# thegedge/StereoReconstruction

Hardware: AMD Instinct MI355X
Metric: Mdisparity-hypotheses/s (WxHxD) (higher is better)
Workload: dtype f64; 1 GPU; C3: synthetic rectified 1920x1080 pair, 256 depth levels, GeodesicWeight r=5; TwoView WTA both directions + cross-check; one pair per GPU; width=1920, height=1080, depth_levels=256, window_radius=5, weights=geodesic, pairs_per_gpu=1, pair_seed_rank0=1592590339, pair_seed_of_rank_r=seed + 0x10000*r, parallelism=single GPU

## Files before the change

stereoreconstruction_amd/csrc/srh_block.hpp:

```cpp
#pragma once

#include <math.h>

#if defined(__HIPCC__)
#include <hip/hip_runtime.h>
#endif
#ifndef SRH_NHD
#if defined(__HIPCC__)
#define SRH_NHD __host__ __device__ __forceinline__
#else
#define SRH_NHD inline
#endif
#endif
#if defined(__HIP_DEVICE_COMPILE__)
#define SRH_SCHED_BARRIER() __builtin_amdgcn_sched_barrier(0)
#define SRH_LDS_WAIT() __builtin_amdgcn_s_waitcnt(0xC07F)
#else
#define SRH_SCHED_BARRIER() do { } while (0)
#define SRH_LDS_WAIT() do { } while (0)
#endif

namespace srh {

template <int WS, int NCB, bool FMA, class Src>
SRH_NHD void block_two_sweeps(const Src src, int ra, int rb, double mL, double tw, double (&sum1)[NCB], double (&sum3)[NCB])
{
	constexpr int NR = NCB + WS - 1;
	static_assert(WS % 2 == 1 && NR % 2 == 0, "odd window, the other view's segment in pairs");
	double r[NR], wv[WS], acc[NCB];
	{
		const auto first = src.row(ra);
#pragma unroll
		for (int m = 0; m < NR/2; ++m) first.r2(m, r[2*m], r[2*m + 1]);
#pragma unroll
		for (int m = 0; m < (WS - 1)/2; ++m) first.w2(m, wv[2*m], wv[2*m + 1]);
		wv[WS - 1] = first.w(WS - 1);
	}
#pragma unroll
	for (int j = 0; j < NCB; ++j) acc[j] = 0.0;
	if (Src::LDS_WAIT) SRH_LDS_WAIT();
#pragma unroll 1
	for (int row = ra; row < rb; ++row) {
		const int seen = src.row_begin(1);
		const auto next = src.row(row + 1 < rb ? row + 1 : ra);
#pragma unroll
		for (int col = 0; col < WS; ++col) {
			if (FMA) {
#pragma unroll
				for (int j = 0; j < NCB; ++j) acc[j] = __builtin_fma(wv[col], r[col + j], acc[j]);
			} else {
				double pr[NCB];
#pragma unroll
				for (int j = 0; j < NCB; ++j) pr[j] = wv[col]*r[col + j];
				SRH_SCHED_BARRIER();
#pragma unroll
				for (int j = 0; j < NCB; ++j) acc[j] += pr[j];
			}
			SRH_SCHED_BARRIER();
			if (col & 1) {
				next.r2(col >> 1, r[col - 1], r[col]);
				next.w2(col >> 1, wv[col - 1], wv[col]);
				SRH_SCHED_BARRIER();
			}
		}
#pragma unroll
		for (int m = (WS - 1)/2; m < NR/2; ++m) next.r2(m, r[2*m], r[2*m + 1]);
		wv[WS - 1] = next.w(WS - 1);
		src.row_end(seen);
	}
	double mR[NCB], s1[NCB], s3[NCB], av[WS];
	{
		const auto first = src.row(ra);
#pragma unroll
		for (int col = 0; col < WS; ++col) av[col] = first.l(col);
	}
#pragma unroll
	for (int j = 0; j < NCB; ++j) { mR[j] = acc[j]/tw; s1[j] = 0.0; s3[j] = 0.0; }
	if (Src::LDS_WAIT) SRH_LDS_WAIT();
#pragma unroll 1
	for (int row = ra; row < rb; ++row) {
		const int seen = src.row_begin(3);
		const auto next = src.row(row + 1 < rb ? row + 1 : ra);
#pragma unroll
		for (int col = 0; col < WS; ++col) {
			const double wt = wv[col];
			if (FMA) {
				const double a = __builtin_fma(wt, av[col], -mL);
				double bb[NCB];
#pragma unroll
				for (int j = 0; j < NCB; ++j) bb[j] = __builtin_fma(wt, r[col + j], -mR[j]);
				SRH_SCHED_BARRIER();
#pragma unroll
				for (int j = 0; j < NCB; ++j) { s1[j] = __builtin_fma(a, bb[j], s1[j]); s3[j] = __builtin_fma(bb[j], bb[j], s3[j]); }
			} else {
				double bb[NCB], u1[NCB], u3[NCB];
				const double pa = wt*av[col];
#pragma unroll
				for (int j = 0; j < NCB; ++j) bb[j] = wt*r[col + j];
				SRH_SCHED_BARRIER();
				const double a = pa - mL;
#pragma unroll
				for (int j = 0; j < NCB; ++j) bb[j] = bb[j] - mR[j];
				SRH_SCHED_BARRIER();
#pragma unroll
				for (int j = 0; j < NCB; ++j) { u1[j] = a*bb[j]; u3[j] = bb[j]*bb[j]; }
				SRH_SCHED_BARRIER();
#pragma unroll
				for (int j = 0; j < NCB; ++j) { s1[j] += u1[j]; s3[j] += u3[j]; }
			}
			SRH_SCHED_BARRIER();
			av[col] = next.l(col);
			if (col & 1) {
				next.r2(col >> 1, r[col - 1], r[col]);
				next.w2(col >> 1, wv[col - 1], wv[col]);
			}
			SRH_SCHED_BARRIER();
		}
#pragma unroll
		for (int m = (WS - 1)/2; m < NR/2; ++m) next.r2(m, r[2*m], r[2*m + 1]);
		wv[WS - 1] = next.w(WS - 1);
		src.row_end(seen);
	}
#pragma unroll
	for (int j = 0; j < NCB; ++j) { sum1[j] = s1[j]; sum3[j] = s3[j]; }
}

template <int WS, int NCB, class Src>
SRH_NHD void block_onepass(const Src src, double mL, double (&Pout)[NCB], double (&Qout)[NCB], double (&Uout)[NCB])
{
	double P[NCB], Q[NCB], U[NCB];
	constexpr int NR = NCB + WS - 1;
	static_assert(WS % 2 == 1 && NR % 2 == 0, "odd window, the other view's segment in pairs");
	double r[NR], q[NR], wv[WS], lv[WS];
	{
		const auto first = src.row(0);
#pragma unroll
		for (int m = 0; m < NR/2; ++m) first.r2(m, r[2*m], r[2*m + 1]);
#pragma unroll
		for (int m = 0; m < (WS - 1)/2; ++m) first.w2(m, wv[2*m], wv[2*m + 1]);
		wv[WS - 1] = first.w(WS - 1);
#pragma unroll
		for (int col = 0; col < WS; ++col) lv[col] = first.l(col);
	}
#pragma unroll
	for (int j = 0; j < NCB; ++j) { P[j] = 0.0; Q[j] = 0.0; U[j] = 0.0; }
	if (Src::LDS_WAIT) SRH_LDS_WAIT();
#pragma unroll 1
	for (int row = 0; row < WS; ++row) {
		const int seen = src.row_begin(4);
		const auto next = src.row(row + 1 < WS ? row + 1 : 0);
#pragma unroll
		for (int k = 0; k < NCB - 1; ++k) q[k] = r[k]*r[k];
#pragma unroll
		for (int col = 0; col < WS; ++col) {
			q[col + NCB - 1] = r[col + NCB - 1]*r[col + NCB - 1];
			const double a = __builtin_fma(wv[col], lv[col], -mL);
			const double c = a*wv[col], d = wv[col]*wv[col];
			SRH_SCHED_BARRIER();
#pragma unroll
			for (int j = 0; j < NCB; ++j) P[j] = __builtin_fma(wv[col], r[col + j], P[j]);
#pragma unroll
			for (int j = 0; j < NCB; ++j) Q[j] = __builtin_fma(c, r[col + j], Q[j]);
#pragma unroll
			for (int j = 0; j < NCB; ++j) U[j] = __builtin_fma(d, q[col + j], U[j]);
			SRH_SCHED_BARRIER();
			lv[col] = next.l(col);
			if (col & 1) {
				next.r2(col >> 1, r[col - 1], r[col]);
				next.w2(col >> 1, wv[col - 1], wv[col]);
			}
			SRH_SCHED_BARRIER();
		}
#pragma unroll
		for (int m = (WS - 1)/2; m < NR/2; ++m) next.r2(m, r[2*m], r[2*m + 1]);
		wv[WS - 1] = next.w(WS - 1);
		src.row_end(seen);
	}
#pragma unroll
	for (int j = 0; j < NCB; ++j) { Pout[j] = P[j]; Qout[j] = Q[j]; Uout[j] = U[j]; }
}

SRH_NHD double two_sweep_finish(double s1, double s2, double s3) { return 255*(1.0 - fabs(s1) / sqrt(s2 * s3)); }

SRH_NHD double rsq_seed(double x)
{
#if defined(__HIP_DEVICE_COMPILE__)
	return __builtin_amdgcn_rsq(x);
#else
	return 1.0/sqrt(x);
#endif
}

SRH_NHD double onepass_finish(double P, double Q, double U, double SA, double itw, double s2, double TT,
                              double sig3, double zmax2, bool &okc)
{
	const double m = P*itw, p2 = P + P;
	const double s3 = __builtin_fma(-m, __builtin_fma(-TT, m, p2), U);
	const double s1 = __builtin_fma(-m, SA, Q);
	const double q3 = __builtin_fma(m, __builtin_fma(TT, m, p2), U);
	const double x = s2*s3;
	const double y0 = rsq_seed(x);
	const double e = __builtin_fma(-(x*y0), y0, 1.0);
	const double y1 = __builtin_fma(y0*e, __builtin_fma(0.375, e, 0.5), y0);
	const bool c1 = s3 >= sig3, c2 = s3*zmax2 >= q3, c3 = __builtin_fabs(e) <= 0x1p-20;
	okc = c1 & c2 & c3;
	return __builtin_fma(-255.0, __builtin_fabs(s1)*y1, 255.0);
}

template <bool CERT, class B = double>
SRH_NHD double block_stored(double v, bool certified, B m_hi, B clamp)
{
	if (CERT) return !certified ? __builtin_nan("") : (v > m_hi ? clamp : v);
	return (v < clamp) ? v : clamp;
}

}
```

stereoreconstruction_amd/csrc/srh_strip.hip:

```cpp
#include "srh_internal.hpp"
#include "srh_geom.hpp"
#include "srh_walk.hpp"
#include "srh_block.hpp"

#include <type_traits>

namespace srh {

#ifdef SRH_EXPERIMENT
__device__ int g_strip_exp_repeat = 1;
void strip_exp_set(int repeat) { (void)hipMemcpyToSymbol(HIP_SYMBOL(g_strip_exp_repeat), &repeat, sizeof(int)); }
#endif

#define ST_TP 32
#define ST_NCB 8
#define ST_CHUNK 320
#define ST_BROWS 1

typedef __attribute__((address_space(3))) void st_lds_void;
typedef __attribute__((address_space(1))) const void st_gbl_void;
typedef __attribute__((address_space(3))) volatile int st_lds_vint;

__global__ void padded_plane_kernel(const double *__restrict__ gray_tv, int W, int H, double *__restrict__ out)
{
	const int SP = padded_stride(W), HP = H + 2*SRH_PADY;
	const size_t n = (size_t)SP*HP;
	const double nan = __builtin_nan("");
	for (size_t k = (size_t)blockIdx.x*blockDim.x + threadIdx.x; k < n; k += (size_t)gridDim.x*blockDim.x) {
		const int x = (int)(k % (size_t)SP) - SRH_PADL, y = (int)(k / (size_t)SP) - SRH_PADY;
		out[k] = (x >= 0 && y >= 0 && x < W && y < H) ? gray_tv[(size_t)y*W + x] : nan;
	}
}

void launch_padded_plane(hipStream_t st, const double *gray_tv, int w, int h, double *out) {
	size_t n = padded_size(w, h);
	size_t b = (n + 255)/256; if (b > 4096) b = 4096;
	hipLaunchKernelGGL(padded_plane_kernel, dim3((unsigned)b), dim3(256), 0, st, gray_tv, w, h, out);
}

__global__ void padded_full_kernel(const double *__restrict__ gray_tv, int W, int H, int R, uint8_t *__restrict__ out)
{
	const int SP = padded_stride(W), HP = H + 2*SRH_PADY;
	const size_t n = (size_t)SP*HP;
	for (size_t k = (size_t)blockIdx.x*blockDim.x + threadIdx.x; k < n; k += (size_t)gridDim.x*blockDim.x) {
		const int x = (int)(k % (size_t)SP) - SRH_PADL, y = (int)(k / (size_t)SP) - SRH_PADY;
		bool ok = x - R >= 0 && y - R >= 0 && x + R < W && y + R < H;
		for (int row = -R; ok && row <= R; ++row)
			for (int col = -R; col <= R; ++col) {
				const double v = gray_tv[(size_t)(y + row)*W + (x + col)];
				ok = ok && (v == v);
			}
		out[k] = ok ? 1 : 0;
	}
}

void launch_padded_full(hipStream_t st, const double *gray_tv, int w, int h, int R, uint8_t *out) {
	size_t n = padded_size(w, h);
	size_t b = (n + 255)/256; if (b > 4096) b = 4096;
	hipLaunchKernelGGL(padded_full_kernel, dim3((unsigned)b), dim3(256), 0, st, gray_tv, w, h, R, out);
}

__global__ void pixel_range_kernel(const ViewDev *__restrict__ views, int ref, int oth, srh_params P, int y0, int nrows,
                                   const double *__restrict__ tnum, int cstride, PixRange *__restrict__ prange,
                                   int ncb, int lanes, int pad, uint32_t *__restrict__ filllist)
{
	const ViewDev &L = views[ref];
	const int W = L.w;
	const size_t q = (size_t)blockIdx.x*blockDim.x + threadIdx.x;
	const bool in = q < (size_t)nrows*W;
	int lo = 0, hi = -1;
	if (in) {
		const int x = (int)(q % W), y = y0 + (int)(q / W);
		if (L.mask[(size_t)y*W + x] == 1) {
			const Ray ray = cam_unproject(L.cam, (x + 0.5) / P.image_scale, (y + 0.5) / P.image_scale);
			pinhole_column_range(ray, L.cam, views[oth], P, tnum, cstride, lo, hi);
		}
		PixRange r; r.lo = lo; r.hi = hi;
		prange[q] = r;
	}
	if (!filllist) return;
	const bool left = in && hi >= lo && dense_cover_hi(lo, hi, ncb, lanes, pad != 0) < hi;
	const unsigned long long m = __ballot(left);
	if (m == 0) return;
	const int lane = (int)(threadIdx.x & 63), leader = __ffsll((long long)m) - 1;
	unsigned base = 0;
	if (lane == leader) base = atomicAdd(&filllist[0], (unsigned)__popcll(m));
	base = (unsigned)__shfl((int)base, leader);
	if (left) filllist[1 + base + (unsigned)__popcll(m & ((1ull << lane) - 1ull))] = (uint32_t)q;
}

void launch_pixel_range(hipStream_t st, const ViewDev *views, int ref, int oth, int width, const srh_params &P,
                        int y0, int nrows, const double *tnum, int cstride, PixRange *prange,
                        int lanes, bool padded, uint32_t *filllist)
{
	const size_t n = (size_t)nrows*width;
	hipLaunchKernelGGL(pixel_range_kernel, dim3((unsigned)((n + 255)/256)), dim3(256), 0, st,
	                   views, ref, oth, P, y0, nrows, tnum, cstride, prange, 8, lanes, padded ? 1 : 0, filllist);
}

int strip_chunk_columns() { return ST_CHUNK; }

struct StripArgs {
	int W, H, y0, nrows;
	const double *wimg;
	const double *pconst;
	const PixRange *prange;
	const double *ref_tvp, *oth_tvp;
	const uint8_t *oth_fullp;
	double *cost; int cstride;
	Counters *cnt;
	int n1, n2;
	int nitems;
	double weight_cutoff, bad_ret, max_color_diff;
	CertBound cb;
	int redo;
};

static void strip_items(StripArgs &a) {
	a.n1 = ((a.nrows*3/4)/16)*16;
	a.n2 = a.n1 + (((a.nrows - a.n1)*2/3)/8)*8;
	const int nseg = a.n1/16 + (a.n2 - a.n1)/8 + (a.nrows - a.n2 + 3)/4;
	a.nitems = nseg*((a.W + ST_TP - 1)/ST_TP);
}

template <int R, int NBUF>
struct StripSmem {
	static constexpr int WS = 2*R + 1;
	static constexpr int T = WS*WS;
	static constexpr int WP = (WS + 1) & ~1;
	static constexpr int WPIX = WS*WP;
	static constexpr int RW = ST_CHUNK + 2*R + ST_NCB + 2;
	static constexpr int LW = (ST_TP + 2*R + 1) & ~1;
	static constexpr int NS = WS + 1;
	static constexpr int FW = (RW + 4 + 15) & ~15;
	static constexpr int NBMAX = ST_CHUNK/ST_NCB + 1;
	static constexpr int GL_CAP = 3072;
	static constexpr int GL_SINGLES = GL_CAP - ST_TP*NBMAX;
	alignas(16) double w[NBUF][WS][ST_TP][WP];
	alignas(16) double rt[NS][RW];
	alignas(16) double rto[NBUF == 2 ? NS : 1][RW];
	alignas(16) double lt[NS][LW];
	alignas(16) double pc[2][ST_TP][SRH_PC];
	alignas(16) PixRange pr[2][ST_TP];
	alignas(16) unsigned char full[2][FW];
	unsigned short glist[GL_CAP];
	int glist_n, gsingle_n;
	int item;
	unsigned long long badcols[ST_CHUNK/64 + 2];
	int simd[8];
	int prog[NBUF == 2 ? 8 : 1][64];
	static_assert(ST_CHUNK <= 512 && ST_TP <= 64, "work-list entry = pixel*512 + column in 16 bits");
	static_assert(RW % 2 == 0 && LW % 2 == 0 && WP % 2 == 0, "16-byte rows");
	static_assert(RW - R + 4 <= SRH_PADR + 1, "padded planes cover every staged piece");
};

__device__ __forceinline__ void st_dma16(const void *src, void *dst, int nbytes, int lane) {
	for (int off = 0; off < nbytes; off += 1024) {
		if (off + lane*16 < nbytes)
			__builtin_amdgcn_global_load_lds((st_gbl_void *)((const char *)src + off + lane*16),
			                                 (st_lds_void *)((char *)dst + off), 16, 0, 0);
	}
}
__device__ __forceinline__ void st_dma4(const void *src, void *dst, int nbytes, int lane) {
	for (int off = 0; off < nbytes; off += 256) {
		if (off + lane*4 < nbytes)
			__builtin_amdgcn_global_load_lds((st_gbl_void *)((const char *)src + off + lane*4),
			                                 (st_lds_void *)((char *)dst + off), 4, 0, 0);
	}
}

template <int R, int NBUF>
__device__ __noinline__ double strip_cost_general(const StripSmem<R, NBUF> &S, int wb, int s0, int i, int rc,
                                                  double weight_cutoff, double bad_ret, double max_color_diff)
{
	typedef StripSmem<R, NBUF> Smem;
	constexpr int WS = Smem::WS, NS = Smem::NS;
	return ncc_select_cost<WS>([&](int row, double *gl, double *gr, double *wt) {
		const int sl = s0 + row >= NS ? s0 + row - NS : s0 + row;
#pragma unroll
		for (int col = 0; col < WS; ++col) { gl[col] = S.lt[sl][i + col]; gr[col] = S.rt[sl][rc + col]; wt[col] = S.w[wb][row][i][col]; }
	}, weight_cutoff, bad_ret, max_color_diff);
}

template <int R, int NBUF>
__device__ __noinline__ void strip_select_block(const StripSmem<R, NBUF> &S, int wb, int s0, int pi, int rc, unsigned store,
                                                double *__restrict__ dst, double weight_cutoff, double bad_ret, double max_color_diff,
                                                int ra, int rb)
{
	typedef StripSmem<R, NBUF> Smem;
	constexpr int WS = Smem::WS, NS = Smem::NS, NCB = ST_NCB, NR = NCB + 2*R;
	double mLs[NCB], mRs[NCB], tws[NCB];
#pragma unroll
	for (int j = 0; j < NCB; ++j) { mLs[j] = 0.0; mRs[j] = 0.0; tws[j] = 0.0; }
#pragma unroll 1
	for (int row = ra; row < rb; ++row) {
		const int sl = s0 + row >= NS ? s0 + row - NS : s0 + row;
		double rr[NR], rv[NR];
		const double2 *rp = reinterpret_cast<const double2 *>((NBUF == 2 && (rc & 1)) ? &S.rto[sl][rc - 1] : &S.rt[sl][rc]);
#pragma unroll
		for (int m = 0; m < NR/2; ++m) { const double2 v = rp[m]; rr[2*m] = v.x; rr[2*m + 1] = v.y; }
#pragma unroll
		for (int m = 0; m < NR; ++m) { const bool okr = rr[m] == rr[m]; rv[m] = okr ? 1.0 : 0.0; rr[m] = okr ? rr[m] : 0.0; }
#pragma unroll
		for (int col = 0; col < WS; ++col) {
			const double gl = S.lt[sl][pi + col], wt = S.w[wb][row][pi][col];
			const bool okl = gl == gl && wt > weight_cutoff;
			const double w0 = okl ? wt : 0.0, pl0 = okl ? wt*gl : 0.0;
#pragma unroll
			for (int j = 0; j < NCB; ++j) {
				mLs[j] += pl0*rv[col + j];
				mRs[j] += w0*rr[col + j];
				tws[j] += w0*rv[col + j];
			}
		}
	}
#pragma unroll
	for (int j = 0; j < NCB; ++j) { mLs[j] /= tws[j]; mRs[j] /= tws[j]; }
	double s1[NCB], s2v[NCB], s3[NCB];
#pragma unroll
	for (int j = 0; j < NCB; ++j) { s1[j] = 0.0; s2v[j] = 0.0; s3[j] = 0.0; }
#pragma unroll 1
	for (int row = ra; row < rb; ++row) {
		const int sl = s0 + row >= NS ? s0 + row - NS : s0 + row;
		double rr[NR], rv[NR];
		const double2 *rp = reinterpret_cast<const double2 *>((NBUF == 2 && (rc & 1)) ? &S.rto[sl][rc - 1] : &S.rt[sl][rc]);
#pragma unroll
		for (int m = 0; m < NR/2; ++m) { const double2 v = rp[m]; rr[2*m] = v.x; rr[2*m + 1] = v.y; }
#pragma unroll
		for (int m = 0; m < NR; ++m) { const bool okr = rr[m] == rr[m]; rv[m] = okr ? 1.0 : 0.0; rr[m] = okr ? rr[m] : 0.0; }
#pragma unroll
		for (int col = 0; col < WS; ++col) {
			const double gl = S.lt[sl][pi + col], wt = S.w[wb][row][pi][col];
			const bool okl = gl == gl && wt > weight_cutoff;
			const double pl = wt*(gl == gl ? gl : 0.0), kl = okl ? 1.0 : 0.0;
#pragma unroll
			for (int j = 0; j < NCB; ++j) {
				const double k = kl*rv[col + j];
				const double a = (pl - mLs[j])*k, bq = (wt*rr[col + j] - mRs[j])*k;
				s1[j] += a*bq;
				s2v[j] += a*a;
				s3[j] += bq*bq;
			}
		}
	}
#pragma unroll
	for (int j = 0; j < NCB; ++j) {
		if ((store >> j) & 1u) {
			double result = bad_ret;
			if (!(tws[j] < 1e-10)) {
				const double v = 255*(1.0 - fabs(s1[j]) / sqrt(s2v[j] * s3[j]));
				result = (v < max_color_diff) ? v : max_color_diff;
			}
			dst[(ptrdiff_t)j*ST_TP] = result;
		}
	}
}

template <int R, int NWV, int NBUF>
struct StripRows {
	typedef StripSmem<R, NBUF> Smem;
	static constexpr bool LDS_WAIT = true;
	Smem &S;
	const double *rbase;
	int s0, wb, i, rc, wv, lane, partner;
	int &prog;
	struct Row {
		const double2 *rp, *wp;
		const double *lp;
		__device__ __forceinline__ void r2(int m, double &a, double &b) const { const double2 v = rp[m]; a = v.x; b = v.y; }
		__device__ __forceinline__ void w2(int m, double &a, double &b) const { const double2 v = wp[m]; a = v.x; b = v.y; }
		__device__ __forceinline__ double w(int col) const { return reinterpret_cast<const double *>(wp)[col]; }
		__device__ __forceinline__ double l(int col) const { return lp[col]; }
	};
	__device__ __forceinline__ Row row(int row) const {
		const int sl = s0 + row >= Smem::NS ? s0 + row - Smem::NS : s0 + row;
		return Row{ reinterpret_cast<const double2 *>(rbase + sl*Smem::RW + rc), reinterpret_cast<const double2 *>(&S.w[wb][row][i][0]), &S.lt[sl][i] };
	}
	__device__ __forceinline__ int row_begin(int units) const {
		int seen = 0;
		if (NWV == 8) {
			prog += units;
			*(st_lds_vint *)&S.prog[wv][lane] = prog;
			seen = *(st_lds_vint *)&S.prog[partner][lane];
		}
		return seen;
	}
	__device__ __forceinline__ void row_end(int seen) const {
		if (NWV == 8) {
			const int ps = __builtin_amdgcn_readfirstlane(seen), pm = __builtin_amdgcn_readfirstlane(prog);
			asm volatile("s_nop 0\n\ts_cmp_gt_i32 %0, %1\n\ts_cbranch_scc1 1f\n\ts_setprio 1\n\ts_branch 2f\n1:\n\ts_setprio 0\n2:"
			             :: "s"(pm), "s"(ps) : "scc");
		}
	}
};

template <int R, int NWV, int NBUF, int AR, bool BORDER>
__global__ __launch_bounds__(NWV*64, 2)
void twoview_strip_cost_kernel(const StripArgs A)
{
	constexpr bool FMA = AR != 0, CERT = AR == 3 || AR == 5, ONEPASS = AR == 5;
	typedef StripSmem<R, NBUF> Smem;
	constexpr int WS = Smem::WS, WP = Smem::WP, WPIX = Smem::WPIX, RW = Smem::RW, LW = Smem::LW, NS = Smem::NS;
	constexpr int NCB = ST_NCB, CHUNK = ST_CHUNK;
	constexpr int NR = NCB + 2*R;
	constexpr int G = 2*NWV;
	constexpr int NT = NWV*64;
	constexpr bool PAD = NBUF == 1;
	static_assert(NR % 2 == 0, "16-byte rows");
	static_assert((NWV == 4 && NBUF == 1) || (NWV == 8 && NBUF == 2), "two forms");
	extern __shared__ __align__(16) unsigned char smem_raw[];
	Smem &S = *reinterpret_cast<Smem *>(smem_raw);
	const Smem &CS = S;

	const int tid = threadIdx.x;
	const int lane = tid & 63;
	const int wv = __builtin_amdgcn_readfirstlane(tid >> 6);
	const int pg = wv & 3;
	const int i = pg*8 + (lane & 7);
	const int g = (lane >> 3) + 8*(wv >> 2);
	const int W = A.W;
	const int tiles_per_row = (W + ST_TP - 1)/ST_TP;
	const int SP = padded_stride(W);
	unsigned n_dev = 0;
	int partner = wv;
	if (NWV == 8) {
		const int simd = (int)__builtin_amdgcn_s_getreg((1 << 11) | (4 << 6) | 4);
		if (lane == 0) S.simd[wv] = simd;
		S.prog[wv][lane] = 0;
		__syncthreads();
		for (int j = 0; j < NWV; ++j) if (j != wv && CS.simd[j] == simd) { partner = j; break; }
		partner = __builtin_amdgcn_readfirstlane(partner);
	}
	int prog = 0;
#ifdef SRH_PROFILE_PHASES
	unsigned long long ph[8] = {0, 0, 0, 0, 0, 0, 0, 0};
	unsigned long long tp = __builtin_readcyclecounter();
	const unsigned long long t_begin = tp;
	unsigned long long n_tiles = 0, n_gen = 0;
#define ST_STAMP(k) do { const unsigned long long tn_ = __builtin_readcyclecounter(); ph[k] += tn_ - tp; tp = tn_; } while (0)
#else
#define ST_STAMP(k) do { } while (0)
#endif

	for (;;) {
		if (tid == 0) S.item = (int)atomicAdd(BORDER ? &A.cnt->strip_ticket_border : &A.cnt->strip_ticket, 1u);
		__syncthreads();
		const int item = __builtin_amdgcn_readfirstlane(S.item);
		ST_STAMP(0);
		if (item >= A.nitems) break;
		int seg = item / tiles_per_row, tx = item - seg*tiles_per_row;
		if (BORDER) {
			const int nseg = (A.n1 + ST_BROWS - 1)/ST_BROWS + (A.nrows - A.n2 + ST_BROWS - 1)/ST_BROWS;
			const int k = item / nseg;
			seg = item - k*nseg;
			tx = k == 0 ? 0 : k == 1 ? tiles_per_row - 1 : k - 1;
		}
		int ya, nh;
		if (BORDER) {
			const int st = (A.n1 + ST_BROWS - 1)/ST_BROWS;
			if (seg < st) { ya = seg*ST_BROWS; nh = A.n1 - ya; }
			else { ya = A.n2 + (seg - st)*ST_BROWS; nh = A.nrows - ya; }
			if (nh > ST_BROWS) nh = ST_BROWS;
		} else {
			const int s16 = A.n1 >> 4, s8 = (A.n2 - A.n1) >> 3;
			if (seg < s16) { ya = seg*16; nh = 16; }
			else if (seg < s16 + s8) { ya = A.n1 + (seg - s16)*8; nh = 8; }
			else { ya = A.n2 + (seg - s16 - s8)*4; nh = 4; }
			if (ya + nh > A.nrows) nh = A.nrows - ya;
		}
		const int x0 = tx*ST_TP;
		const int x = x0 + i;
		int cs = 0, rowbase = 0;

		auto issue_tile_inputs = [&](int r, int buf, int wb, bool consts, bool windows) {
			const size_t px0 = (size_t)r*W + x0;
			if (consts && wv == 0) st_dma16(A.pconst + px0*SRH_PC, &S.pc[buf][0][0], ST_TP*SRH_PC*8, lane);
			if (consts && wv == 1) st_dma4(A.prange + px0, &S.pr[buf][0], ST_TP*8, lane);
			if (windows) {
				const double *wt = A.wimg + ((size_t)r*tiles_per_row + tx)*(size_t)(ST_TP*WPIX);
				if (NBUF == 1) {
					for (int a = 0; a < WS; ++a)
						st_dma16(wt + (size_t)a*(ST_TP*WP) + pg*8*WP, &S.w[wb][a][pg*8][0], 8*WP*8, lane);
				} else {
					constexpr int NBYTES = ST_TP*WPIX*8;
					for (int off = wv*1024; off < NBYTES; off += NWV*1024)
						if (off + lane*16 < NBYTES)
							__builtin_amdgcn_global_load_lds((st_gbl_void *)((const char *)wt + off + lane*16),
							                                 (st_lds_void *)((char *)&S.w[wb][0][0][0] + off), 16, 0, 0);
				}
			}
		};
		auto issue_row = [&](int yy, int sl) {
			const double *src = A.oth_tvp + (size_t)(yy + SRH_PADY)*SP + (cs - R + SRH_PADL);
			if (wv < 3) { if (wv*1024 + lane*16 < RW*8) __builtin_amdgcn_global_load_lds((st_gbl_void *)((const char *)src + wv*1024 + lane*16),
			                                                                              (st_lds_void *)((char *)&S.rt[sl][0] + wv*1024), 16, 0, 0); }
			else if (wv == 3) st_dma16(A.ref_tvp + (size_t)(yy + SRH_PADY)*SP + (x0 - R + SRH_PADL), &S.lt[sl][0], LW*8, lane);
			else if (NBUF == 2 && wv < 7) {
				const int pc = wv - 4;
				if (pc*1024 + lane*16 < RW*8) __builtin_amdgcn_global_load_lds((st_gbl_void *)((const char *)(src + 1) + pc*1024 + lane*16),
				                                                                (st_lds_void *)((char *)&S.rto[sl][0] + pc*1024), 16, 0, 0);
			}
		};
		static_assert(RW*8 <= 3*1024, "three pieces per row of the other view");
		auto issue_full = [&](int fy, int fb) {
			const size_t a0 = (size_t)(fy + SRH_PADY)*SP + (size_t)(cs + SRH_PADL);
			if (!BORDER && wv == NWV - 1) st_dma4(A.oth_fullp + (a0 & ~(size_t)3), &S.full[fb][0], (RW + 4 + 3) & ~3, lane);
		};

		bool first = true;
		for (int r = ya; r < ya + nh; ++r) {
			const int y = A.y0 + r;
			const int cur = (r - ya) & 1, nxt = cur ^ 1;
			const int wcur = NBUF == 2 ? cur : 0, wnxt = NBUF == 2 ? nxt : 0;
			const bool has_next = r + 1 < ya + nh;
			if (first) issue_tile_inputs(r, cur, wcur, true, true);
			asm volatile("s_waitcnt vmcnt(0)" ::: "memory");
			ST_STAMP(1);
			__builtin_amdgcn_s_barrier();
			ST_STAMP(2);

			int cmin, cmax, cmin_raw;
			{
				const int pi = lane & 31;
				const PixRange q = CS.pr[cur][pi];
				int lo = q.lo, hi = q.hi;
				if (x0 + pi >= W) { lo = 0; hi = -1; }
				if (hi >= lo) hi = dense_cover_hi(lo, hi, NCB, G, PAD);
				int mn = hi >= lo ? lo : 2147483647, mx = hi >= lo ? hi : -2147483647;
#define ST_ROR(v, n) __builtin_amdgcn_update_dpp(0, (v), 0x120 + (n), 0xf, 0xf, false)
#pragma unroll
				for (int d = 8; d >= 1; d >>= 1) {
					const int on = d == 8 ? ST_ROR(mn, 8) : d == 4 ? ST_ROR(mn, 4) : d == 2 ? ST_ROR(mn, 2) : ST_ROR(mn, 1);
					const int ox = d == 8 ? ST_ROR(mx, 8) : d == 4 ? ST_ROR(mx, 4) : d == 2 ? ST_ROR(mx, 2) : ST_ROR(mx, 1);
					mn = on < mn ? on : mn; mx = ox > mx ? ox : mx;
				}
#undef ST_ROR
				{
					const int m0 = __builtin_amdgcn_readlane(mn, 0), m1 = __builtin_amdgcn_readlane(mn, 16);
					const int x0_ = __builtin_amdgcn_readlane(mx, 0), x1_ = __builtin_amdgcn_readlane(mx, 16);
					cmin_raw = m0 < m1 ? m0 : m1;
					cmax = x0_ > x1_ ? x0_ : x1_;
				}
				cmin = cmin_raw & ~1;
			}
			const bool any = cmin_raw <= cmax;
			if (first || (any && (cmin < cs || cmax > cs + CHUNK - 1))) {
				if (!first) __builtin_amdgcn_s_barrier();
				cs = any ? cmin : 0;
				rowbase = y - R;
				for (int rr = 0; rr < WS; ++rr) issue_row(y - R + rr, rr);
				issue_full(y, cur);
				asm volatile("s_waitcnt vmcnt(0)" ::: "memory");
				__builtin_amdgcn_s_barrier();
			}
			if (any && cmax > cs + CHUNK - 1) {
				if (tid == 0) atomicAdd(&A.cnt->strip_overflow, 1ull);
				cmax = cs + CHUNK - 1;
			}
			first = false;
			const int s0 = (y - R - rowbase) % NS;
			if (has_next) {
				issue_row(y + R + 1, (y + R + 1 - rowbase) % NS);
				issue_full(y + 1, nxt);
				issue_tile_inputs(r + 1, nxt, wnxt, true, NBUF == 2);
			}
			const int foff = BORDER ? 0 : (int)(((size_t)(y + SRH_PADY)*SP + (size_t)(cs + SRH_PADL)) & 3);
			const unsigned char *rfull = &CS.full[cur][foff];
			const int bra = BORDER ? (y < R ? R - y : 0) : 0;
			const int brb = BORDER ? (y + R > A.H - 2 ? WS - (y + R - (A.H - 2)) : WS) : WS;
			if (BORDER) {
				unsigned char *cok = &S.full[nxt][0];
				for (int k = tid; k < RW; k += NT) {
					bool ok = true;
					for (int row = bra; row < brb; ++row) {
						const int sl = s0 + row >= NS ? s0 + row - NS : s0 + row;
						const double v = CS.rt[sl][k];
						ok = ok && v == v;
					}
					cok[k] = ok ? 1 : 0;
				}
				if (g == 0) {
					const PixelConstants c = pixel_constants<WS, false>([&](int row, double *gl, double *wt) {
						const int sl = s0 + row >= NS ? s0 + row - NS : s0 + row;
						for (int col = 0; col < WS; ++col) { gl[col] = CS.lt[sl][i + col]; wt[col] = CS.w[wcur][row][i][col]; }
					}, A.weight_cutoff, x < W, bra, brb);
					S.pc[cur][i][0] = c.mL; S.pc[cur][i][1] = c.tw; S.pc[cur][i][2] = c.s2; S.pc[cur][i][3] = c.all ? 1.0/c.tw : 0.0;
				}
				__syncthreads();
				for (int k = tid; k < CHUNK + NCB; k += NT) {
					bool ok = true;
					for (int d = 0; d < WS; ++d) ok = ok && cok[k + d] != 0;
					S.full[cur][k] = ok ? 1 : 0;
				}
				__syncthreads();
			}

			bool need_general = false;
			{
				const int pi = lane & 31;
				const PixRange q = CS.pr[cur][pi];
				const bool live = x0 + pi < W && q.hi >= q.lo;
				bool bad = live && !(CS.pc[cur][pi][3] != 0.0);
#pragma unroll
				for (int it = 0; it < (CHUNK + 63)/64 + 1; ++it) {
					const int k = it*64 + lane, c = cs + k;
					const bool colbad = k < CHUNK + NCB && rfull[k] == 0;
					if (colbad && c >= cmin_raw && c <= cmax) bad = true;
					const unsigned long long m = __ballot(colbad);
					if (wv == 0 && lane == 0) S.badcols[it] = m;
				}
				need_general = __any(bad) != 0;
			}

			if (NWV == 8) { prog = 0; *(st_lds_vint *)&S.prog[wv][lane] = 0; __builtin_amdgcn_s_setprio(1); }
			int e_min, e_max;
			{
				const PixRange q = CS.pr[cur][i];
				e_min = q.lo; e_max = q.hi;
				if (x >= W) { e_min = 0; e_max = -1; }
				if (e_max >= e_min) e_max = dense_cover_hi(e_min, e_max, NCB, G, PAD);
			}
			const bool lall = CS.pc[cur][i][3] != 0.0;
			const double sig3 = CERT ? A.cb.sigma3(CS.pc[cur][i][2]) : 0.0;
			const bool pix_exact = CERT && A.redo && !(sig3 < __builtin_inf());
			const size_t tile = (size_t)r*tiles_per_row + tx;
			ST_STAMP(3);
			if (e_max >= e_min) {
				const int lo = e_min > cs ? e_min : cs;
				const int hi = e_max < cs + CHUNK - 1 ? e_max : cs + CHUNK - 1;
				const int lo_e = PAD ? (lo & ~1) : lo;
				const int nblocks = hi >= lo ? (hi - lo_e + NCB)/NCB : 0;
				double *crow = A.cost + tile*(size_t)A.cstride*ST_TP + i;
#ifdef SRH_EXPERIMENT
				const int exp_rep = g_strip_exp_repeat;
				for (int rep = 0; rep < exp_rep; ++rep)
#endif
				for (int b = g; b < (lall ? nblocks : 0); b += G) {
					const int c0 = lo_e + b*NCB;
					const int rc = c0 - cs;
					const double *rbase = (!PAD && (rc & 1)) ? &CS.rto[0][0] - 1 : &CS.rt[0][0];
					StripRows<R, NWV, NBUF> rows{ S, rbase, s0, wcur, i, rc, wv, lane, partner, prog };
					unsigned vm = 0;
#pragma unroll
					for (int j = 0; j < NCB; ++j) {
						const int c = c0 + j;
						vm |= (c >= lo && c <= hi && rfull[rc + j] != 0) ? 1u << j : 0u;
					}
					const bool fast = vm != 0;
					n_dev += __builtin_popcount(vm);
					bool bad_blk = false;
					auto two_sweeps = [&](auto fma_c, auto cert_c) {
						constexpr bool FMAc = decltype(fma_c)::value, CERTc = decltype(cert_c)::value;
						const double mL = CS.pc[cur][i][0], tw = CS.pc[cur][i][1], s2 = CS.pc[cur][i][2];
						double s1[NCB], s3[NCB];
						block_two_sweeps<WS, NCB, FMAc>(rows, BORDER ? bra : 0, BORDER ? brb : WS, mL, tw, s1, s3);
#pragma unroll
						for (int j = 0; j < NCB; ++j) {
							const int c = c0 + j;
							if (c >= lo && c <= hi && rfull[rc + j] != 0) {
								const bool okc = s3[j] >= sig3;
								if (CERTc && !okc && A.redo) bad_blk = true;
								crow[(size_t)(c - e_min)*ST_TP] = block_stored<CERTc, const double &>(two_sweep_finish(s1[j], s2, s3[j]), okc, A.cb.m_hi, A.max_color_diff);
							}
							__builtin_amdgcn_sched_barrier(0);
						}
					};
					if (BORDER) {
						if (fast) two_sweeps(std::false_type(), std::false_type());
					} else if (fast && ONEPASS && !pix_exact) {
						const double mL = CS.pc[cur][i][0], itw = CS.pc[cur][i][3], s2 = CS.pc[cur][i][2];
						double P_[NCB], Q_[NCB], U_[NCB];
						block_onepass<WS, NCB>(rows, mL, P_, Q_, U_);
						constexpr double TT = (double)(WS*WS);
						const double zmax2 = A.cb.zmax2, mhi = A.cb.m_hi, mcd = A.max_color_diff, SA = CS.pc[cur][i][4];
						const bool redo = A.redo != 0;
#pragma unroll
						for (int j = 0; j < NCB; ++j) {
							bool okc;
							const double v = onepass_finish(P_[j], Q_[j], U_[j], SA, itw, s2, TT, sig3, zmax2, okc);
							const bool st = (vm >> j) & 1u;
							bad_blk |= st & !okc & redo;
							if (st) crow[(size_t)(c0 + j - e_min)*ST_TP] = block_stored<true>(v, okc, mhi, mcd);
						}
					} else if (fast && !ONEPASS && !pix_exact) two_sweeps(std::integral_constant<bool, FMA>(), std::integral_constant<bool, CERT>());
					if (!BORDER && fast && CERT && (pix_exact || bad_blk)) two_sweeps(std::false_type(), std::false_type());
				}
			}
			if (NWV == 8) __builtin_amdgcn_s_setprio(2);
			ST_STAMP(4);
			if (need_general) {
				if (tid == 0) { S.glist_n = 0; S.gsingle_n = 0; }
				__syncthreads();
				for (int p = tid; p < ST_TP*Smem::NBMAX; p += NT) {
					const int pi = p / Smem::NBMAX, b = p % Smem::NBMAX;
					const PixRange q = CS.pr[cur][pi];
					int qlo = q.lo, qhi = q.hi;
					if (x0 + pi >= W) { qlo = 0; qhi = -1; }
					if (qhi >= qlo) qhi = dense_cover_hi(qlo, qhi, NCB, G, PAD);
					if (qhi > cs + CHUNK - 1) qhi = cs + CHUNK - 1;
					if (qhi < qlo) continue;
					const int c0 = (PAD ? (qlo & ~1) : qlo) + b*NCB;
					if (c0 > qhi) continue;
					const bool pall = CS.pc[cur][pi][3] != 0.0;
					unsigned need = 0xffu;
					if (qlo > c0) need &= 0xffu << (qlo - c0);
					if (c0 + NCB - 1 > qhi) need &= 0xffu >> (c0 + NCB - 1 - qhi);
					if (pall) {
						const int rc = c0 - cs, wd = rc >> 6, sh = rc & 63;
						unsigned long long bits = CS.badcols[wd] >> sh;
						if (sh) bits |= CS.badcols[wd + 1] << (64 - sh);
						need &= (unsigned)bits;
					}
					if (!need) continue;
					bool as_block = __builtin_popcount(need) == NCB;
					if (!as_block) {
						const int at = atomicAdd(&S.gsingle_n, __builtin_popcount(need));
						if (at + __builtin_popcount(need) <= Smem::GL_SINGLES) {
							int k = 0;
#pragma unroll
							for (int j = 0; j < NCB; ++j)
								if ((need >> j) & 1u) { S.glist[Smem::GL_CAP - 1 - (at + k)] = (unsigned short)(pi*512 + (c0 + j - cs)); ++k; }
						} else {
							for (int k = at; k < at + __builtin_popcount(need) && k < Smem::GL_SINGLES; ++k) S.glist[Smem::GL_CAP - 1 - k] = 0xffffu;
							as_block = true;
						}
					}
					if (as_block) S.glist[atomicAdd(&S.glist_n, 1)] = (unsigned short)(pi*64 + b);
				}
				__syncthreads();
				ST_STAMP(5);
#ifdef SRH_PROFILE_PHASES
				++n_gen;
#endif
				const int nblk = S.glist_n;
				const int nsingle = S.gsingle_n < Smem::GL_SINGLES ? S.gsingle_n : Smem::GL_SINGLES;
				for (int q = tid; q < nblk; q += NT) {
					const int pi = S.glist[q] >> 6, b = S.glist[q] & 63;
					const PixRange pq = CS.pr[cur][pi];
					int qhi = dense_cover_hi(pq.lo, pq.hi, NCB, G, PAD);
					if (qhi > cs + CHUNK - 1) qhi = cs + CHUNK - 1;
					const int c0 = (PAD ? (pq.lo & ~1) : pq.lo) + b*NCB;
					const bool pall = CS.pc[cur][pi][3] != 0.0;
					unsigned store = 0;
#pragma unroll
					for (int j = 0; j < NCB; ++j) {
						const int c = c0 + j;
						if (c >= pq.lo && c <= qhi && !(pall && rfull[c - cs])) { store |= 1u << j; ++n_dev; }
					}
					strip_select_block<R, NBUF>(CS, wcur, s0, pi, c0 - cs, store,
					                            A.cost + (tile*(size_t)A.cstride)*ST_TP + (ptrdiff_t)(c0 - pq.lo)*ST_TP + pi,
					                            A.weight_cutoff, A.bad_ret, A.max_color_diff,
					                            y < R ? R - y : 0, y + R > A.H - 2 ? WS - (y + R - (A.H - 2)) : WS);
				}
				ST_STAMP(6);
				for (int q = tid; q < nsingle; q += NT) {
					const unsigned short e = S.glist[Smem::GL_CAP - 1 - q];
					if (e == 0xffffu) continue;
					const int pi = e >> 9, k = e & 511;
					++n_dev;
					A.cost[(tile*(size_t)A.cstride + (size_t)(cs + k - CS.pr[cur][pi].lo))*ST_TP + pi] =
						strip_cost_general<R, NBUF>(CS, wcur, s0, pi, k, A.weight_cutoff, A.bad_ret, A.max_color_diff);
				}
				ST_STAMP(7);
				__syncthreads();
			}
			if (NBUF == 1 && has_next) issue_tile_inputs(r + 1, nxt, 0, false, true);
			ST_STAMP(2);
#ifdef SRH_PROFILE_PHASES
			++n_tiles;
#endif
		}
	}
	block_count_add(&A.cnt->n_eval_device, n_dev);
#ifdef SRH_PROFILE_PHASES
	if (lane == 0) {
		for (int k = 0; k < 8; ++k) atomicAdd(&A.cnt->dbg_phase[k], ph[k]);
		atomicAdd(&A.cnt->dbg_blocks, n_tiles);
		atomicAdd(&A.cnt->dbg_cycles, n_gen);
		for (int k = 0; k < 8; ++k) atomicAdd(&A.cnt->dbg_wave[8*k + (wv & 7)], ph[k]);
		atomicAdd(&A.cnt->dbg_total_cycles, (unsigned long long)(__builtin_readcyclecounter() - t_begin));
		atomicAdd(&A.cnt->dbg_waves, 1ull);
	}
#endif
#undef ST_STAMP
}

template <int R, int NWV, int NBUF, int AR, bool BORDER>
static void launch_strip_variant(hipStream_t st, const StripArgs &a, int num_cus)
{
	typedef StripSmem<R, NBUF> Smem;
	size_t lds = sizeof(Smem);
	(void)hipFuncSetAttribute((const void *)twoview_strip_cost_kernel<R, NWV, NBUF, AR, BORDER>,
	                          hipFuncAttributeMaxDynamicSharedMemorySize, (int)lds);
	int grid = num_cus*(NBUF == 2 ? 1 : 2);
	if (grid > a.nitems) grid = a.nitems;
	if (grid < 1) grid = 1;
	hipLaunchKernelGGL((twoview_strip_cost_kernel<R, NWV, NBUF, AR, BORDER>), dim3((unsigned)grid), dim3(NWV*64), lds, st, a);
}

template <int R, int NWV, int NBUF>
static void launch_strip_arith(hipStream_t st, const StripArgs &a, int num_cus, int arith)
{
	const int tiles_per_row = (a.W + ST_TP - 1)/ST_TP;
	const int t = std::min(std::max(R - a.y0, 0), a.nrows);
	const int b = std::min(std::max(a.H - 1 - R - a.y0, t), a.nrows);
	if (b > t) {
		StripArgs m = a;
		const size_t tiles = (size_t)t*tiles_per_row;
		m.y0 = a.y0 + t; m.nrows = b - t;
		m.wimg = a.wimg + tiles*(ST_TP*StripSmem<R, NBUF>::WPIX);
		m.pconst = a.pconst + (size_t)t*a.W*SRH_PC;
		m.prange = a.prange + (size_t)t*a.W;
		m.cost = a.cost + tiles*(size_t)a.cstride*ST_TP;
		strip_items(m);
		if (arith == 5) launch_strip_variant<R, NWV, NBUF, 5, false>(st, m, num_cus);
		else if (arith == 3) launch_strip_variant<R, NWV, NBUF, 3, false>(st, m, num_cus);
		else if (arith == 1) launch_strip_variant<R, NWV, NBUF, 1, false>(st, m, num_cus);
		else launch_strip_variant<R, NWV, NBUF, 0, false>(st, m, num_cus);
	}
	if (t > 0 || b < a.nrows) {
		StripArgs e = a;
		e.n1 = t; e.n2 = b;
		e.nitems = ((t + ST_BROWS - 1)/ST_BROWS + (a.nrows - b + ST_BROWS - 1)/ST_BROWS)*tiles_per_row;
		launch_strip_variant<R, NWV, NBUF, 0, true>(st, e, num_cus);
	}
}

int strip_block_lanes(int cstride, int form) {
	if (form == 4) return 8;
	if (form == 8) return 16;
	return cstride > 16*ST_NCB ? 16 : 8;
}

bool launch_twoview_strip_cost(hipStream_t st, const ViewDev *views, int ref, int oth, int width, int height,
                               const srh_params &P, int y0, int nrows, const double *wimg, const double *pconst,
                               const PixRange *prange, const double *ref_tvp, const double *oth_tvp,
                               const uint8_t *oth_fullp, double *cost, int cstride, Counters *cnt, int arith, int num_cus,
                               int lanes, bool raw)
{
	(void)views; (void)ref; (void)oth;
	StripArgs a;
	a.W = width; a.H = height; a.y0 = y0; a.nrows = nrows;
	a.wimg = wimg; a.pconst = pconst; a.prange = prange;
	a.ref_tvp = ref_tvp; a.oth_tvp = oth_tvp; a.oth_fullp = oth_fullp;
	a.cost = cost; a.cstride = cstride; a.cnt = cnt;
	a.weight_cutoff = P.weight_cutoff; a.bad_ret = P.bad_ret; a.max_color_diff = P.max_color_diff;
	a.cb = cert_bound(P);
	a.redo = raw ? 0 : 1;
	const bool wide = lanes == 16;
	switch (P.window_radius) {
	case 5:
		if (wide) launch_strip_arith<5, 8, 2>(st, a, num_cus, arith); else launch_strip_arith<5, 4, 1>(st, a, num_cus, arith);
		return true;
	case 2:
		if (wide) launch_strip_arith<2, 8, 2>(st, a, num_cus, arith); else launch_strip_arith<2, 4, 1>(st, a, num_cus, arith);
		return true;
	default: return false;
	}
}

}
```

Measured before the change: 48490 Mhyp/s.

## Precompute per-tap left coefficients in LDS and drop odd-offset row copy

For the 8-wave double-buffered one-pass path, a cooperative pass now precomputes per-tap coefficients (w*l - mL)*w into a new LDS array, and the inner loop reads them instead of recomputing from the left-view tile. The shifted copy of the other view's rows (rto), previously DMA'd so odd offsets could use 16-byte loads, is removed. Odd-offset reads now use scalar 8-byte volatile LDS reads. This trades fewer DMA transfers and inner-loop arithmetic for an extra barrier-synchronised precompute pass and narrower LDS reads, which may cost bandwidth.

```diff
diff --git a/stereoreconstruction_amd/csrc/srh_block.hpp b/stereoreconstruction_amd/csrc/srh_block.hpp
--- a/stereoreconstruction_amd/csrc/srh_block.hpp
+++ b/stereoreconstruction_amd/csrc/srh_block.hpp
@@ -174,6 +174,60 @@
 #pragma unroll
 		for (int m = (WS - 1)/2; m < NR/2; ++m) next.r2(m, r[2*m], r[2*m + 1]);
 		wv[WS - 1] = next.w(WS - 1);
+		src.row_end(seen);
+	}
+#pragma unroll
+	for (int j = 0; j < NCB; ++j) { Pout[j] = P[j]; Qout[j] = Q[j]; Uout[j] = U[j]; }
+}
+
+template <int WS, int NCB, class Src>
+SRH_NHD void block_onepass_taps(const Src src, double (&Pout)[NCB], double (&Qout)[NCB], double (&Uout)[NCB])
+{
+	double P[NCB], Q[NCB], U[NCB];
+	constexpr int NR = NCB + WS - 1;
+	static_assert(WS % 2 == 1 && NR % 2 == 0, "odd window, the other view's segment in pairs");
+	double r[NR], q[NR], wv[WS], cv[WS];
+	{
+		const auto first = src.row(0);
+#pragma unroll
+		for (int m = 0; m < NR/2; ++m) first.r2(m, r[2*m], r[2*m + 1]);
+#pragma unroll
+		for (int m = 0; m < (WS - 1)/2; ++m) { first.w2(m, wv[2*m], wv[2*m + 1]); first.c2(m, cv[2*m], cv[2*m + 1]); }
+		wv[WS - 1] = first.w(WS - 1);
+		cv[WS - 1] = first.c(WS - 1);
+	}
+#pragma unroll
+	for (int j = 0; j < NCB; ++j) { P[j] = 0.0; Q[j] = 0.0; U[j] = 0.0; }
+	if (Src::LDS_WAIT) SRH_LDS_WAIT();
+#pragma unroll 1
+	for (int row = 0; row < WS; ++row) {
+		const int seen = src.row_begin(4);
+		const auto next = src.row(row + 1 < WS ? row + 1 : 0);
+#pragma unroll
+		for (int k = 0; k < NCB - 1; ++k) q[k] = r[k]*r[k];
+#pragma unroll
+		for (int col = 0; col < WS; ++col) {
+			q[col + NCB - 1] = r[col + NCB - 1]*r[col + NCB - 1];
+			const double d = wv[col]*wv[col];
+			SRH_SCHED_BARRIER();
+#pragma unroll
+			for (int j = 0; j < NCB; ++j) P[j] = __builtin_fma(wv[col], r[col + j], P[j]);
+#pragma unroll
+			for (int j = 0; j < NCB; ++j) Q[j] = __builtin_fma(cv[col], r[col + j], Q[j]);
+#pragma unroll
+			for (int j = 0; j < NCB; ++j) U[j] = __builtin_fma(d, q[col + j], U[j]);
+			SRH_SCHED_BARRIER();
+			if (col & 1) {
+				next.r2(col >> 1, r[col - 1], r[col]);
+				next.w2(col >> 1, wv[col - 1], wv[col]);
+				next.c2(col >> 1, cv[col - 1], cv[col]);
+			}
+			SRH_SCHED_BARRIER();
+		}
+#pragma unroll
+		for (int m = (WS - 1)/2; m < NR/2; ++m) next.r2(m, r[2*m], r[2*m + 1]);
+		wv[WS - 1] = next.w(WS - 1);
+		cv[WS - 1] = next.c(WS - 1);
 		src.row_end(seen);
 	}
 #pragma unroll
diff --git a/stereoreconstruction_amd/csrc/srh_strip.hip b/stereoreconstruction_amd/csrc/srh_strip.hip
--- a/stereoreconstruction_amd/csrc/srh_strip.hip
+++ b/stereoreconstruction_amd/csrc/srh_strip.hip
@@ -20,6 +20,9 @@
 typedef __attribute__((address_space(3))) void st_lds_void;
 typedef __attribute__((address_space(1))) const void st_gbl_void;
 typedef __attribute__((address_space(3))) volatile int st_lds_vint;
+typedef __attribute__((address_space(3))) const volatile double st_lds_vdouble;
+
+__device__ __forceinline__ double st_lds_read8(const double *p) { return *(st_lds_vdouble *)p; }
 
 __global__ void padded_plane_kernel(const double *__restrict__ gray_tv, int W, int H, double *__restrict__ out)
 {
@@ -138,7 +141,7 @@
 	static constexpr int GL_SINGLES = GL_CAP - ST_TP*NBMAX;
 	alignas(16) double w[NBUF][WS][ST_TP][WP];
 	alignas(16) double rt[NS][RW];
-	alignas(16) double rto[NBUF == 2 ? NS : 1][RW];
+	alignas(16) double c[NBUF == 2 ? WS : 1][NBUF == 2 ? ST_TP : 1][WP];
 	alignas(16) double lt[NS][LW];
 	alignas(16) double pc[2][ST_TP][SRH_PC];
 	alignas(16) PixRange pr[2][ST_TP];
@@ -196,9 +199,14 @@
 	for (int row = ra; row < rb; ++row) {
 		const int sl = s0 + row >= NS ? s0 + row - NS : s0 + row;
 		double rr[NR], rv[NR];
-		const double2 *rp = reinterpret_cast<const double2 *>((NBUF == 2 && (rc & 1)) ? &S.rto[sl][rc - 1] : &S.rt[sl][rc]);
-#pragma unroll
-		for (int m = 0; m < NR/2; ++m) { const double2 v = rp[m]; rr[2*m] = v.x; rr[2*m + 1] = v.y; }
+		if (NBUF == 2) {
+#pragma unroll
+			for (int m = 0; m < NR; ++m) rr[m] = st_lds_read8(&S.rt[sl][rc + m]);
+		} else {
+			const double2 *rp = reinterpret_cast<const double2 *>(&S.rt[sl][rc]);
+#pragma unroll
+			for (int m = 0; m < NR/2; ++m) { const double2 v = rp[m]; rr[2*m] = v.x; rr[2*m + 1] = v.y; }
+		}
 #pragma unroll
 		for (int m = 0; m < NR; ++m) { const bool okr = rr[m] == rr[m]; rv[m] = okr ? 1.0 : 0.0; rr[m] = okr ? rr[m] : 0.0; }
 #pragma unroll
@@ -223,9 +231,14 @@
 	for (int row = ra; row < rb; ++row) {
 		const int sl = s0 + row >= NS ? s0 + row - NS : s0 + row;
 		double rr[NR], rv[NR];
-		const double2 *rp = reinterpret_cast<const double2 *>((NBUF == 2 && (rc & 1)) ? &S.rto[sl][rc - 1] : &S.rt[sl][rc]);
-#pragma unroll
-		for (int m = 0; m < NR/2; ++m) { const double2 v = rp[m]; rr[2*m] = v.x; rr[2*m + 1] = v.y; }
+		if (NBUF == 2) {
+#pragma unroll
+			for (int m = 0; m < NR; ++m) rr[m] = st_lds_read8(&S.rt[sl][rc + m]);
+		} else {
+			const double2 *rp = reinterpret_cast<const double2 *>(&S.rt[sl][rc]);
+#pragma unroll
+			for (int m = 0; m < NR/2; ++m) { const double2 v = rp[m]; rr[2*m] = v.x; rr[2*m + 1] = v.y; }
+		}
 #pragma unroll
 		for (int m = 0; m < NR; ++m) { const bool okr = rr[m] == rr[m]; rv[m] = okr ? 1.0 : 0.0; rr[m] = okr ? rr[m] : 0.0; }
 #pragma unroll
@@ -261,20 +274,27 @@
 	typedef StripSmem<R, NBUF> Smem;
 	static constexpr bool LDS_WAIT = true;
 	Smem &S;
-	const double *rbase;
 	int s0, wb, i, rc, wv, lane, partner;
 	int &prog;
 	struct Row {
-		const double2 *rp, *wp;
+		const double *rp;
+		const double2 *wp;
 		const double *lp;
-		__device__ __forceinline__ void r2(int m, double &a, double &b) const { const double2 v = rp[m]; a = v.x; b = v.y; }
+		const double2 *cp;
+		__device__ __forceinline__ void c2(int m, double &a, double &b) const { const double2 v = cp[m]; a = v.x; b = v.y; }
+		__device__ __forceinline__ double c(int col) const { return reinterpret_cast<const double *>(cp)[col]; }
+		__device__ __forceinline__ void r2(int m, double &a, double &b) const {
+			if (NBUF == 2) { a = st_lds_read8(rp + 2*m); b = st_lds_read8(rp + 2*m + 1); }
+			else { const double2 v = reinterpret_cast<const double2 *>(rp)[m]; a = v.x; b = v.y; }
+		}
 		__device__ __forceinline__ void w2(int m, double &a, double &b) const { const double2 v = wp[m]; a = v.x; b = v.y; }
 		__device__ __forceinline__ double w(int col) const { return reinterpret_cast<const double *>(wp)[col]; }
 		__device__ __forceinline__ double l(int col) const { return lp[col]; }
 	};
 	__device__ __forceinline__ Row row(int row) const {
 		const int sl = s0 + row >= Smem::NS ? s0 + row - Smem::NS : s0 + row;
-		return Row{ reinterpret_cast<const double2 *>(rbase + sl*Smem::RW + rc), reinterpret_cast<const double2 *>(&S.w[wb][row][i][0]), &S.lt[sl][i] };
+		return Row{ &S.rt[sl][rc], reinterpret_cast<const double2 *>(&S.w[wb][row][i][0]), &S.lt[sl][i],
+		            reinterpret_cast<const double2 *>(&S.c[NBUF == 2 ? row : 0][NBUF == 2 ? i : 0][0]) };
 	}
 	__device__ __forceinline__ int row_begin(int units) const {
 		int seen = 0;
@@ -306,6 +326,7 @@
 	constexpr int G = 2*NWV;
 	constexpr int NT = NWV*64;
 	constexpr bool PAD = NBUF == 1;
+	constexpr bool TAPS = NBUF == 2 && ONEPASS && !BORDER;
 	static_assert(NR % 2 == 0, "16-byte rows");
 	static_assert((NWV == 4 && NBUF == 1) || (NWV == 8 && NBUF == 2), "two forms");
 	extern __shared__ __align__(16) unsigned char smem_raw[];
@@ -395,11 +416,6 @@
 			if (wv < 3) { if (wv*1024 + lane*16 < RW*8) __builtin_amdgcn_global_load_lds((st_gbl_void *)((const char *)src + wv*1024 + lane*16),
 			                                                                              (st_lds_void *)((char *)&S.rt[sl][0] + wv*1024), 16, 0, 0); }
 			else if (wv == 3) st_dma16(A.ref_tvp + (size_t)(yy + SRH_PADY)*SP + (x0 - R + SRH_PADL), &S.lt[sl][0], LW*8, lane);
-			else if (NBUF == 2 && wv < 7) {
-				const int pc = wv - 4;
-				if (pc*1024 + lane*16 < RW*8) __builtin_amdgcn_global_load_lds((st_gbl_void *)((const char *)(src + 1) + pc*1024 + lane*16),
-				                                                                (st_lds_void *)((char *)&S.rto[sl][0] + pc*1024), 16, 0, 0);
-			}
 		};
 		static_assert(RW*8 <= 3*1024, "three pieces per row of the other view");
 		auto issue_full = [&](int fy, int fb) {
@@ -512,6 +528,22 @@
 				need_general = __any(bad) != 0;
 			}
 
+			if (TAPS) {
+				constexpr int HP = WP/2, NPAIR = WS*ST_TP*HP;
+				for (int e = tid; e < NPAIR; e += NT) {
+					const int row = e/(ST_TP*HP), pe = e - row*(ST_TP*HP), pi = pe/HP, col = 2*(pe - pi*HP);
+					const int sl = s0 + row >= NS ? s0 + row - NS : s0 + row;
+					const double mL = CS.pc[cur][pi][0];
+					const double2 wt = *reinterpret_cast<const double2 *>(&CS.w[wcur][row][pi][col]);
+					const bool two = col + 1 < WS;
+					const double l0 = CS.lt[sl][pi + col], l1 = two ? CS.lt[sl][pi + col + 1] : 0.0;
+					double2 cc;
+					cc.x = __builtin_fma(wt.x, l0, -mL)*wt.x;
+					cc.y = two ? __builtin_fma(wt.y, l1, -mL)*wt.y : 0.0;
+					*reinterpret_cast<double2 *>(&S.c[row][pi][col]) = cc;
+				}
+				__syncthreads();
+			}
 			if (NWV == 8) { prog = 0; *(st_lds_vint *)&S.prog[wv][lane] = 0; __builtin_amdgcn_s_setprio(1); }
 			int e_min, e_max;
 			{
@@ -538,8 +570,7 @@
 				for (int b = g; b < (lall ? nblocks : 0); b += G) {
 					const int c0 = lo_e + b*NCB;
 					const int rc = c0 - cs;
-					const double *rbase = (!PAD && (rc & 1)) ? &CS.rto[0][0] - 1 : &CS.rt[0][0];
-					StripRows<R, NWV, NBUF> rows{ S, rbase, s0, wcur, i, rc, wv, lane, partner, prog };
+					StripRows<R, NWV, NBUF> rows{ S, s0, wcur, i, rc, wv, lane, partner, prog };
 					unsigned vm = 0;
 #pragma unroll
 					for (int j = 0; j < NCB; ++j) {
@@ -570,7 +601,8 @@
 					} else if (fast && ONEPASS && !pix_exact) {
 						const double mL = CS.pc[cur][i][0], itw = CS.pc[cur][i][3], s2 = CS.pc[cur][i][2];
 						double P_[NCB], Q_[NCB], U_[NCB];
-						block_onepass<WS, NCB>(rows, mL, P_, Q_, U_);
+						if (TAPS) block_onepass_taps<WS, NCB>(rows, P_, Q_, U_);
+						else block_onepass<WS, NCB>(rows, mL, P_, Q_, U_);
 						constexpr double TT = (double)(WS*WS);
 						const double zmax2 = A.cb.zmax2, mhi = A.cb.m_hi, mcd = A.max_color_diff, SA = CS.pc[cur][i][4];
 						const bool redo = A.redo != 0;
@@ -689,6 +721,7 @@
 static void launch_strip_variant(hipStream_t st, const StripArgs &a, int num_cus)
 {
 	typedef StripSmem<R, NBUF> Smem;
+	static_assert(sizeof(Smem) <= (NBUF == 2 ? 160 : 80)*1024, "a compute unit's 160 KB of LDS: one 8-wave workgroup or two 4-wave ones");
 	size_t lds = sizeof(Smem);
 	(void)hipFuncSetAttribute((const void *)twoview_strip_cost_kernel<R, NWV, NBUF, AR, BORDER>,
 	                          hipFuncAttributeMaxDynamicSharedMemorySize, (int)lds);
```

Result: faster. 49490 Mhyp/s (median of 6 runs) (+2.1%).
